# wwood/CoverM

Measured on AMD Instinct MI355X. Metric: aligned reads/s through coverm contig (mean trimmed_mean covered_fraction variance), higher is better.
Workload: dtype i32 depth / u64 sums / f32 estimators

## Files before the change

coverm_amd/csrc/pileup_kernels.hip.h:

```cpp
#pragma once
#include <hip/hip_runtime.h>
#include <stdint.h>

#define HSTC_FN __host__ __device__ __forceinline__
#include "hist_stats_core.h"
#include "scan_ops.hip.h"

namespace covk {

typedef unsigned long long u64;
typedef unsigned int u32;

constexpr u32 F_POS_UNSORTED = 1u;
constexpr u32 RW_SINGLE = 0u, RW_DOUBLE = 1u, RW_COMPLEX = 2u, RW_BUCKET = 3u;
constexpr u32 FAST_MAX_CAND = 8191u;
constexpr u32 TILE_F_GENERIC = 1u, TILE_F_SLOW = 2u;
constexpr u32 CX_MIN_OPS = 16;

struct DevContig {
    u64 n_primary, n_pass, n_nonsupp, sum_nm, sum_indel;
    double id_primary, id_nonsupp;
    u64 sum_d, sum_d2, cov_win, cov_full, proc_win;
    u64 hist_off;
    u32 first_rec, last_rec;
// ... 1029 lines not shown
    const u32 k0 = generic ? 0u : (rs + ID_CH - 1) / ID_CH, k1 = generic ? 0u : re / ID_CH;
    if (k0 >= k1) { serial(rs, re, true, true); }
    else {
        serial(rs, k0 * ID_CH, true, true);
        for (u32 kb = k0; kb < k1; kb += 64) {
            const u32 kk = kb + (u32)lane;
            IdChunk x;
            if (kk < k1) x = ch[kk]; else { x.tp = x.tn = 0; x.ep = x.en = ID_SERIAL; x.flags = 15u; }
            const u32 nb = min(64u, k1 - kb);
            auto run_stream = [&](double &S, const int e_l, const u64 t_l, const bool bad_l, const bool is_p) {
                u32 q = 0;
                while (q < nb) {
                    const u64 bits = (u64)__double_as_longlong(S);
                    const int e_cur = (int)((bits >> 52) & 0x7ff) - 1023;
                    const u64 m = (bits & 0xfffffffffffffull) | (1ull << 52);
                    const bool in_range = (u32)lane >= q && (u32)lane < nb;
                    const u64 P = wave_incl_scan_u64(in_range ? t_l : 0ull);
                    const bool fits = in_range && !bad_l && !(bits >> 63) && e_l == e_cur && t_l < (1ull << 53) &&
                                      P < (1ull << 53) && m + P < (1ull << 53);
                    const u64 failm = __ballot(in_range && !fits);
                    const u32 jstar = failm ? (u32)(__ffsll((long long)failm) - 1) : nb;
                    if (jstar > q) {
                        const u64 T = bcast_u64(P, (int)(jstar - 1));
                        S = __longlong_as_double((long long)((bits & 0xfff0000000000000ull) | ((m + T) & 0xfffffffffffffull)));
                    }
                    if (jstar < nb) serial((kb + jstar) * ID_CH, (kb + jstar + 1) * ID_CH, is_p, !is_p);
                    q = jstar + 1;
                }
            };
            if (identp != nullptr) run_stream(Sp, x.ep, x.tp, (x.flags & (1u | 4u)) != 0u, true);
            if (identn != nullptr) run_stream(Sn, x.en, x.tn, (x.flags & (2u | 8u)) != 0u, false);
        }
        serial(k1 * ID_CH, re, true, true);
    }
    if (lane == 0) { C->id_primary = Sp; C->id_nonsupp = Sn; }
}

__device__ __attribute__((noinline)) void hist_add_overflow(u32 *arena, u64 hoff, u32 hcap, DevGlobal *g, u32 d, u32 x) {
    if (d <= hcap) atomicAdd(&arena[hoff + d], x);
    else atomicOr(&g->internal_error, 1u);
}

struct PileupArgs {
    const u32 *tile_contig, *tile_start;
    const uint4 *desc;
    const uint2 *runs;
    const uint2 *cx_runs;
    Records r;
    DevContig *ctg;
    DevGlobal *g;
    u32 *hist_arena;
    u64 excl;
    int32_t *depth_out;
    const u64 *depth_off;
    u32 tile_base;
};


__device__ __forceinline__ void lds_fence() { asm volatile("s_waitcnt lgkmcnt(0)" ::: "memory"); }

constexpr int STREAM_TW = 1024, STREAM_HB = 512, STREAM_CAP = 512;

template <bool WANT_HIST, bool WRITE_DEPTH>
__global__ __launch_bounds__(256) void k_pileup_stream(PileupArgs a, u32 n_tiles, u32 chunk_tiles,
                                                       const u32 *__restrict__ tile_list, const u32 *__restrict__ n_list) {
    if (tile_list != nullptr) n_tiles = *n_list;
    constexpr int TW = STREAM_TW, HBW = STREAM_HB, CAP = STREAM_CAP, ROWS = TW / 64;
    extern __shared__ __attribute__((aligned(16))) char smem[];
    const int lane = threadIdx.x & 63, w = threadIdx.x >> 6;
    int *tile = reinterpret_cast<int *>(smem + (size_t)w * (TW * 4 + HBW * 4));
    u32 *lhist = reinterpret_cast<u32 *>(tile + TW);
    int4 *t4 = reinterpret_cast<int4 *>(tile);
    int2 *ent = reinterpret_cast<int2 *>(tile);
    const u32 wave_id = blockIdx.x * 4u + (u32)w, n_waves = gridDim.x * 4u;
    if (WANT_HIST) {
#pragma unroll
        for (int b = lane; b < HBW; b += 64) lhist[b] = 0u;
    }
    u64 sum_d = 0, sum_d2 = 0, proc_win = 0;
    u32 cov_w = 0, cov_f = 0, mn = 0xffffffffu, mx = 0;
    u32 cov_o = 0;
    u32 hbound = 0;
    int cur_c = -1;
    u64 hoff = 0; u32 hcap = 0;
    const u64 excl = a.excl;

    auto hist_add = [&](u32 d, u32 x) {
        if (__builtin_expect(d < (u32)HBW, 1)) atomicAdd(&lhist[d], x);
        else hist_add_overflow(a.hist_arena, hoff, hcap, a.g, d, x);
    };
    auto flush = [&]() {
        if (WANT_HIST) {
            if (cur_c >= 0) {
                lds_fence();
                for (u32 b = (u32)lane; b <= hbound; b += 64) {
                    const u32 x = lhist[b];
                    if (x) { atomicAdd(&a.hist_arena[hoff + b], x); lhist[b] = 0u; }
                }
                lds_fence();
                if (__any(cov_o != 0u)) {
                    const u32 co = wave_sum_u32(cov_o);
                    if (lane == 0) atomicAdd(&a.ctg[cur_c].cov_out, co);
                }
            }
            cov_o = 0; hbound = 0;
            return;
        }
        if (cur_c >= 0) {
            const u64 s1 = wave_sum_u64(sum_d), s2 = wave_sum_u64(sum_d2);
            const u32 c1 = wave_sum_u32(cov_w), c2 = wave_sum_u32(cov_f);
            const u32 m1 = wave_min_u32(mn), m2 = wave_max_u32(mx);
            DevContig *C = &a.ctg[cur_c];
            if (lane == 0) {
                if (s1) atomicAdd(&C->sum_d, s1);
                if (s2) atomicAdd(&C->sum_d2, s2);
                if (c1) atomicAdd(&C->cov_win, (u64)c1);
                if (c2) atomicAdd(&C->cov_full, (u64)c2);
                if (proc_win) {
                    atomicAdd(&C->proc_win, proc_win);
                    atomicMin(&C->min_d, m1);
                    atomicMax(&C->max_d, m2);
                }
            }
        }
        sum_d = sum_d2 = 0; proc_win = 0; cov_w = cov_f = 0; mn = 0xffffffffu; mx = 0;
    };

    auto load_runs = [&](const uint4 &d, uint2 &r0, uint2 &r1) {
        const u32 i0 = d.x + (u32)lane, i1 = i0 + 64u;
        r0 = i0 < d.y ? a.runs[i0] : make_uint2(0u, 0u);
        r1 = i1 < d.y ? a.runs[i1] : make_uint2(0u, 0u);
    };
    const u32 n_chunks = (n_tiles + chunk_tiles - 1) / chunk_tiles;
    u32 ch = wave_id < n_chunks ? wave_id : 0xffffffffu;
    while (ch != 0xffffffffu) {
        const u32 ch_next = ch + n_waves < n_chunks ? ch + n_waves : 0xffffffffu;
        const u32 t0 = a.tile_base + ch * chunk_tiles, t1 = a.tile_base + min((ch + 1) * chunk_tiles, n_tiles);
        for (u32 tq = t0; tq < t1; tq++) {
            const u32 t = tile_list != nullptr ? tile_list[tq] : tq;
            const uint4 ds = a.desc[2 * (size_t)t], dC1 = a.desc[2 * (size_t)t + 1];
            uint2 rw0, rw1;
            load_runs(ds, rw0, rw1);
            const u32 c = dC1.x, lo = dC1.y, L = ds.z;
            const u64 dbase = (WRITE_DEPTH && a.depth_off != nullptr) ? a.depth_off[c] : 0ull;
            const u32 cxo = dC1.z, cxn = dC1.w;
            if (ds.x >= ds.y && cxn == 0u) continue;
            const bool generic = ds.w & 1u;
            if ((int)c != cur_c) {
                flush();
                cur_c = (int)c;
                if (WANT_HIST) { hoff = a.ctg[c].hist_off; hcap = a.ctg[c].hist_cap; }
            }
            const u32 tlen_t = min((u32)TW, L - lo);
#pragma unroll
            for (int k = 0; k < TW / 256; k++) t4[k * 64 + lane] = make_int4(0, 0, 0, 0);
            lds_fence();
            const u32 hi = lo + TW;
            auto add_run = [&](u32 s, u32 e) {
                if (s < hi && e > lo) {
                    const u32 s0 = s > lo ? s - lo : 0u;
                    atomicAdd(&tile[s0], 1);
                    if (e < hi) atomicAdd(&tile[e - lo], -1);
                }
            };
            auto apply = [&](const uint2 rw, u32 i) {
                if (rw.y == 0u) return;
                if (generic && a.r.tid[i] != (int)c) return;
                const u32 type = rw.y >> 30;
                if (type <= RW_DOUBLE) {
                    const bool dbl = type == RW_DOUBLE;
                    const u32 l1 = dbl ? (rw.y & 1023u) : rw.y;
                    add_run(rw.x, rw.x + l1);
                    if (dbl) {
                        const u32 s2 = rw.x + l1 + ((rw.y >> 10) & 255u);
                        add_run(s2, s2 + ((rw.y >> 18) & 1023u));
                    }
                } else if (type == RW_COMPLEX) {
                    u32 cursor = (u32)a.r.pos[i];
                    const u32 c0 = a.r.cigar_off[i], c1 = a.r.cigar_off[i + 1];
                    for (u32 k = c0; k < c1; k++) {
                        const u32 wd = a.r.cigar[k];
                        const u32 op = wd & 15u, len = wd >> 4;
                        if (op == 0u || op == 7u || op == 8u) { add_run(cursor, cursor + len); cursor += len; }
                        else if (op == 2u || op == 3u) cursor += len;
                    }
                }
            };
            apply(rw0, ds.x + (u32)lane);
            apply(rw1, ds.x + 64u + (u32)lane);
            for (u32 i = ds.x + 128u + (u32)lane; i < ds.y; i += 64) apply(a.runs[i], i);
            for (u32 j = (u32)lane; j < cxn; j += 64) { const uint2 q = a.cx_runs[(u64)cxo + j]; add_run(q.x, q.y); }
            lds_fence();
            int x[ROWS];
            u32 E = 0;
#pragma unroll
            for (int j = 0; j < ROWS; j++) x[j] = tile[j * 64 + lane];
#pragma unroll
            for (int j = 0; j < ROWS; j++) E += (u32)__popcll(__ballot(x[j] != 0));
            const bool has_win = 2 * excl < (u64)L;
            const u32 ws = has_win ? (u32)excl : 0u, we = has_win ? (u32)(L - excl) : 0u;
            const u32 wst = max(ws, lo), wet = min(we, lo + tlen_t);
            const bool win_any = has_win && wst < wet;
            if (!WANT_HIST && win_any) proc_win += (u64)(wet - wst);
            if (WANT_HIST) hbound = max(hbound, min(ds.y - ds.x + cxn, (u32)HBW - 1u));

            if (!WRITE_DEPTH && E <= (u32)CAP) {
                u32 base = 0;
#pragma unroll
                for (int j = 0; j < ROWS; j++) {
                    const u64 m = __ballot(x[j] != 0);
                    if (x[j] != 0) {
                        const u32 rank = __builtin_amdgcn_mbcnt_hi((u32)(m >> 32), __builtin_amdgcn_mbcnt_lo((u32)m, 0u));
                        ent[base + rank] = make_int2(j * 64 + lane, x[j]);
                    }
                    base += (u32)__popcll(m);
                }
                lds_fence();
                const u32 wl0 = win_any ? wst - lo : 0u, wl1 = win_any ? wet - lo : 0u;
                if (lane == 0) {
                    const u32 en = min(E ? (u32)ent[0].x : tlen_t, tlen_t);
                    const u32 a1 = min(en, wl1);
                    if (a1 > wl0) { if (WANT_HIST) hist_add(0u, a1 - wl0); else mn = 0u; }
                }
                int carry = 0;
                u32 s1t = 0, s2t = 0;
                for (u32 e0 = 0; e0 < E; e0 += 64) {
                    const u32 e = e0 + (u32)lane;
                    const bool live = e < E;
                    const int2 en = live ? ent[e] : make_int2(0, 0);
                    const u32 nxt = (e + 1 < E) ? (u32)ent[e + 1].x : tlen_t;
                    const int inc = wave_incl_scan(en.y);
                    const int d = carry + inc;
                    carry += __builtin_amdgcn_readlane(inc, 63);
                    const u32 du = (u32)d;
                    const bool small = !__any(live && du >= 1024u);
                    if (live) {
                        const u32 s = min((u32)en.x, tlen_t), t_ = min(nxt, tlen_t);
                        const u32 a0 = max(s, wl0), a1 = min(t_, wl1);
                        if (WANT_HIST) {
                            const u32 len = a1 > a0 ? a1 - a0 : 0u;
                            if (d > 0) cov_o += (t_ - s) - len;
                            if (len) hist_add(du, len);
                        } else {
                            if (d > 0) cov_f += t_ - s;
                            if (a1 > a0) {
                                const u32 len = a1 - a0;
                                if (small) { s1t += __umul24(du, len); s2t += __umul24(__umul24(du, du), len); }
                                else { sum_d += (u64)du * len; sum_d2 += (u64)du * du * len; }
                                if (d > 0) cov_w += len;
                                mn = min(mn, du); mx = max(mx, du);
                            }
                        }
                    }
                }
                sum_d += s1t; sum_d2 += s2t;
            } else {
                int carry = 0;
#pragma unroll
                for (int j = 0; j < ROWS; j++) {
                    const int inc = wave_incl_scan(x[j]);
                    const int d = carry + inc;
                    carry += __builtin_amdgcn_readlane(inc, 63);
                    const u32 p = lo + (u32)(j * 64 + lane);
                    const u32 du = (u32)d;
                    if (p < L) {
                        if (WRITE_DEPTH) a.depth_out[dbase + p] = d;
                        const bool in_w = win_any && p >= wst && p < wet;
                        if (WANT_HIST) {
                            if (in_w) {
                                const u32 rel = p - wst;
                                if (x[j] != 0 && rel) { hist_add((u32)(d - x[j]), rel); hist_add(du, 0u - rel); }
                                if (p == wet - 1) hist_add(du, wet - wst);
                            } else cov_o += d > 0;
                        } else {
                            cov_f += d > 0;
                            if (in_w) {
                                sum_d += du;
                                sum_d2 += (u64)du * du;
                                cov_w += d > 0;
                                mn = min(mn, du); mx = max(mx, du);
                            }
                        }
                    }
                }
            }
        }
        flush();
        cur_c = -1;
        ch = ch_next;
    }
}

constexpr size_t pileup_stream_smem_bytes() { return (size_t)4 * ((size_t)STREAM_TW * 4 + STREAM_HB * 4); }

constexpr int FAST_TW = 1024, FAST_HB = 512;
constexpr int FAST_HB7 = 384;
constexpr size_t pileup_fast_smem_bytes(bool hist, int hb = FAST_HB, int tables = 2) { return (size_t)4 * ((size_t)FAST_TW * 2 * tables + (hist ? (size_t)hb * 4 : 0)); }

typedef short v2i16 __attribute__((ext_vector_type(2)));
typedef __attribute__((address_space(3))) u32 lds_u32_t;
__device__ __forceinline__ u32 lds_addr_of(const u32 *p) { return (u32)(uintptr_t)(lds_u32_t *)p; }
__device__ __forceinline__ void lds_atomic_add(u32 addr, u32 x) { (void)__hip_atomic_fetch_add((lds_u32_t *)(uintptr_t)addr, x, __ATOMIC_RELAXED, __HIP_MEMORY_SCOPE_WORKGROUP); }

template <bool WANT_HIST, int HB, int TABLES>
__device__ __forceinline__ void pileup_fast_body(const PileupArgs &a, u32 n_tiles, u32 chunk_tiles) {
    constexpr int TW = FAST_TW, HBW = HB;
    constexpr int DS = TABLES == 1 ? 2 : 0;
    constexpr size_t WB = (size_t)TW * 2 * TABLES + (WANT_HIST ? (size_t)HBW * 4 : 0);
    extern __shared__ __attribute__((aligned(16))) char smem[];
    const int lane = threadIdx.x & 63, w = threadIdx.x >> 6;
    u32 *S = reinterpret_cast<u32 *>(smem + (size_t)w * WB);
    u32 *E = TABLES == 2 ? S + TW / 2 : S;
    u32 *lhist = S + (TW / 2) * TABLES;
    uint4 *S4 = reinterpret_cast<uint4 *>(S), *E4 = reinterpret_cast<uint4 *>(E);
    const u32 wave_id = (u32)__builtin_amdgcn_readfirstlane((int)(blockIdx.x * 4u + (u32)w)), n_waves = gridDim.x * 4u;
    if (WANT_HIST) {
#pragma unroll
        for (int b = lane; b < HBW; b += 64) lhist[b] = 0u;
    }
    u64 sum_d = 0, sum_d2 = 0, proc_win = 0;
    u32 cov_w = 0, cov_f = 0, mn = 0xffffffffu, mx = 0;
    u32 cov_o = 0;
    int cur_c = -1;
    u64 hoff = 0; u32 hcap = 0;
    const u64 excl = a.excl;
    u32 hbound = 0;
    auto drain = [&]() {
        lds_fence();
        for (u32 b = (u32)lane; b <= hbound; b += 64) {
            const u32 x = lhist[b];
            if (x) { atomicAdd(&a.hist_arena[hoff + b], x); lhist[b] = 0u; }
        }
        lds_fence();
        hbound = 0;
    };

    auto hist_add = [&](u32 d, u32 x) {
        if (__builtin_expect(d < (u32)HBW, 1)) atomicAdd(&lhist[d], x);
        else hist_add_overflow(a.hist_arena, hoff, hcap, a.g, d, x);
    };
    auto flush = [&]() {
        if (WANT_HIST) {
            if (cur_c >= 0) {
                drain();
                if (__any(cov_o != 0u)) {
                    const u32 co = wave_sum_u32_dpp(cov_o);
                    if (lane == 0) atomicAdd(&a.ctg[cur_c].cov_out, co);
                }
            }
            cov_o = 0; hbound = 0;
            return;
        }
        if (cur_c >= 0) {
            const bool narrow = !__any((sum_d | sum_d2) >> 50);
            const u64 s1 = narrow ? wave_sum_u56(sum_d) : wave_sum_u64(sum_d), s2 = narrow ? wave_sum_u56(sum_d2) : wave_sum_u64(sum_d2);
            const u32 c1 = wave_sum_u32_dpp(cov_w), c2 = wave_sum_u32_dpp(cov_f);
            const u32 m1 = wave_min_u32_dpp(mn), m2 = wave_max_u32_dpp(mx);
            DevContig *C = &a.ctg[cur_c];
            if (lane == 0) {
                if (s1) atomicAdd(&C->sum_d, s1);
                if (s2) atomicAdd(&C->sum_d2, s2);
                if (c1) atomicAdd(&C->cov_win, (u64)c1);
                if (c2) atomicAdd(&C->cov_full, (u64)c2);
                if (proc_win) {
                    atomicAdd(&C->proc_win, proc_win);
                    atomicMin(&C->min_d, m1);
                    atomicMax(&C->max_d, m2);
                }
            }
        }
        sum_d = sum_d2 = 0; proc_win = 0; cov_w = cov_f = 0; mn = 0xffffffffu; mx = 0;
    };
    auto load_runs = [&](const uint4 &d, uint2 &r0, uint2 &r1) {
        const u32 i0 = d.x + (u32)lane, i1 = i0 + 64u;
        r0 = i0 < d.y ? a.runs[i0] : make_uint2(0u, 0u);
        r1 = i1 < d.y ? a.runs[i1] : make_uint2(0u, 0u);
    };
    const u32 n_chunks = (n_tiles + chunk_tiles - 1) / chunk_tiles;
    if (wave_id >= n_chunks) return;
    u32 ch = wave_id;
    u32 t = ch * chunk_tiles, t_end = min(t + chunk_tiles, n_tiles);
    uint4 ds = a.desc[2 * (size_t)(a.tile_base + t)], dC1 = a.desc[2 * (size_t)(a.tile_base + t) + 1];
    uint2 rw0, rw1;
    load_runs(ds, rw0, rw1);
    for (;;) {
        u32 tn = t + 1, tn_end = t_end, chn = ch;
        bool chunk_end = false;
        if (tn >= t_end) {
            chunk_end = true;
            chn = ch + n_waves;
            tn = chn < n_chunks ? chn * chunk_tiles : 0xffffffffu;
            tn_end = chn < n_chunks ? min(tn + chunk_tiles, n_tiles) : 0u;
        }
        const bool have_next = tn != 0xffffffffu;
        uint4 nds = make_uint4(0u, 0u, 0u, 0u), ndC1 = make_uint4(0u, 0u, 0u, 0u);
        if (have_next) { nds = a.desc[2 * (size_t)(a.tile_base + tn)]; ndC1 = a.desc[2 * (size_t)(a.tile_base + tn) + 1]; }

        const u32 c = dC1.x, lo = dC1.y, L = ds.z, cxo = dC1.z, cxn = dC1.w;
        const bool live = (ds.x < ds.y || cxn != 0u) && !(ds.w & TILE_F_SLOW);
        uint4 sv0, sv1, ev0, ev1;
        if (live) {
            if ((int)c != cur_c) {
                flush();
                cur_c = (int)c;
                if (WANT_HIST) { hoff = a.ctg[c].hist_off; hcap = a.ctg[c].hist_cap; }
            }
            const u32 zb = TABLES == 2 ? 0u : 0x80008000u;
            const uint4 z4 = make_uint4(zb, zb, zb, zb);
            S4[2 * lane] = z4; S4[2 * lane + 1] = z4;
            if (TABLES == 2) { E4[2 * lane] = z4; E4[2 * lane + 1] = z4; }
            asm volatile("" ::: "memory");
            const u32 hi = lo + TW;
            auto add_run = [&](u32 s, u32 e) {
                if (s < hi && e > lo) {
                    const u32 s0 = s > lo ? s - lo : 0u;
                    atomicAdd(&S[s0 >> 1], (1u << DS) << ((s0 & 1u) << 4));
                    if (e < hi) {
                        const u32 e0 = e - lo;
                        if (TABLES == 2) atomicAdd(&E[e0 >> 1], 1u << ((e0 & 1u) << 4)); else atomicSub(&E[e0 >> 1], (1u << DS) << ((e0 & 1u) << 4));
                    }
                }
            };
            auto apply = [&](const uint2 rw, u32 i) {
                if (rw.y == 0u) return;
                const u32 type = rw.y >> 30;
                if (type <= RW_DOUBLE) {
                    const bool dbl = type == RW_DOUBLE;
                    const u32 l1 = dbl ? (rw.y & 1023u) : rw.y;
                    add_run(rw.x, rw.x + l1);
                    if (dbl) {
                        const u32 s2 = rw.x + l1 + ((rw.y >> 10) & 255u);
                        add_run(s2, s2 + ((rw.y >> 18) & 1023u));
                    }
                } else if (type == RW_COMPLEX) {
                    u32 cursor = (u32)a.r.pos[i];
                    const u32 c0 = a.r.cigar_off[i], c1 = a.r.cigar_off[i + 1];
                    for (u32 k = c0; k < c1; k++) {
                        const u32 wd = a.r.cigar[k];
                        const u32 op = wd & 15u, len = wd >> 4;
                        if (op == 0u || op == 7u || op == 8u) { add_run(cursor, cursor + len); cursor += len; }
                        else if (op == 2u || op == 3u) cursor += len;
                    }
                }
            };
            apply(rw0, ds.x + (u32)lane);
            if (ds.y - ds.x > 64u) {
                apply(rw1, ds.x + 64u + (u32)lane);
                for (u32 i = ds.x + 128u + (u32)lane; i < ds.y; i += 64) apply(a.runs[i], i);
            }
            for (u32 j = (u32)lane; j < cxn; j += 64) { const uint2 q = a.cx_runs[(u64)cxo + j]; add_run(q.x, q.y); }
            asm volatile("" ::: "memory");
            sv0 = S4[2 * lane]; sv1 = S4[2 * lane + 1];
            if (TABLES == 2) { ev0 = E4[2 * lane]; ev1 = E4[2 * lane + 1]; }
        }
        uint2 nrw0 = make_uint2(0u, 0u), nrw1 = make_uint2(0u, 0u);
        if (have_next) load_runs(nds, nrw0, nrw1);

        if (live) {
            const u32 sw[8] = {sv0.x, sv0.y, sv0.z, sv0.w, sv1.x, sv1.y, sv1.z, sv1.w};
            u32 ew[8] = {0u, 0u, 0u, 0u, 0u, 0u, 0u, 0u};
            if (TABLES == 2) { ew[0] = ev0.x; ew[1] = ev0.y; ew[2] = ev0.z; ew[3] = ev0.w; ew[4] = ev1.x; ew[5] = ev1.y; ew[6] = ev1.z; ew[7] = ev1.w; }
            v2i16 dl[8];
#pragma unroll
            for (int k = 0; k < 8; k++) dl[k] = TABLES == 2 ? __builtin_bit_cast(v2i16, sw[k]) - __builtin_bit_cast(v2i16, ew[k]) : __builtin_bit_cast(v2i16, sw[k] ^ 0x80008000u);
            int net = 0;
            const v2i16 one2 = {1, 1};
#pragma unroll
            for (int k = 0; k < 8; k++) net = __builtin_amdgcn_sdot2(dl[k], one2, net, false);
            int d = wave_incl_scan(net) - net;

            const bool has_win = 2 * excl < (u64)L;
            const u32 tlen_t = min((u32)TW, L - lo);
            const u32 ws = has_win ? (u32)excl : 0u, we = has_win ? (u32)(L - excl) : 0u;
            const u32 wst = max(ws, lo), wet = min(we, lo + tlen_t);
            const bool win_any = has_win && wst < wet;
            if (!WANT_HIST && win_any) proc_win += (u64)(wet - wst);
            const bool interior = has_win && lo >= ws && lo + (u32)TW <= we;
            const u32 cand = ds.y - ds.x + cxn;
            const bool fast_tile = interior && cand < (u32)HBW;
            if (WANT_HIST) hbound = max(hbound, min(cand, (u32)HBW - 1u));
            if (WANT_HIST && fast_tile) {
                u32 seg0 = 0;
                u32 da = lds_addr_of(lhist) + ((u32)d << (2 - DS));
#pragma unroll
                for (int j = 0; j < 16; j++) {
                    const int dj = (j & 1) ? (int)dl[j >> 1].y : (int)dl[j >> 1].x;
                    if (j > 0 && dj != 0) { lds_atomic_add(da, (u32)j - seg0); seg0 = (u32)j; }
                    da += (u32)(dj << (2 - DS));
                }
                lds_atomic_add(da, 16u - seg0);
            } else if (WANT_HIST && cand < (u32)HBW) {
                const u32 p0 = lo + 16u * (u32)lane;
                const u32 wa = win_any ? min(max(wst, p0) - p0, 16u) : 0u, wb = win_any ? min(max(wet, p0) - p0, 16u) : 0u;
                const u32 le = min(max(L, p0) - p0, 16u);
                u32 seg0 = 0, covm = 0;
                const u32 da0 = lds_addr_of(lhist);
                u32 da = da0 + ((u32)d << (2 - DS));
#pragma unroll
                for (int j = 0; j < 16; j++) {
                    const int dj = (j & 1) ? (int)dl[j >> 1].y : (int)dl[j >> 1].x;
                    if (j > 0 && dj != 0) {
                        const u32 s_ = max(seg0, wa), e_ = min((u32)j, wb);
                        if (e_ > s_) lds_atomic_add(da, e_ - s_);
                        seg0 = (u32)j;
                    }
                    da += (u32)(dj << (2 - DS));
                    covm = covm + covm + (da != da0 ? 1u : 0u);
                }
                {
                    const u32 s_ = max(seg0, wa);
                    if (wb > s_) lds_atomic_add(da, wb - s_);
                }
                const u32 in_ctg = 0xffffu & ~(0xffffu >> le), in_win = (0xffffu >> wa) & ~(0xffffu >> wb);
                cov_o += (u32)__popc(covm & in_ctg & ~in_win);
            } else if (WANT_HIST) {
                const u32 p0 = lo + 16u * (u32)lane;
                u32 seg0 = 0;
                bool seg_open = false;
#pragma unroll 4
                for (int j = 0; j < 16; j++) {
                    const int dj = (j & 1) ? (int)dl[j >> 1].y : (int)dl[j >> 1].x;
                    const u32 p = p0 + (u32)j;
                    const bool in_w = win_any && p >= wst && p < wet;
                    if (seg_open && (dj != 0 || !in_w)) { hist_add((u32)d >> DS, (u32)j - seg0); seg_open = false; }
                    d += dj;
                    if (in_w) { if (!seg_open) { seg_open = true; seg0 = (u32)j; } }
                    else if (p < L) cov_o += d != 0 ? 1u : 0u;
                }
                if (seg_open) hist_add((u32)d >> DS, 16u - seg0);
            } else if (fast_tile) {
                u32 s1t = 0, s2t = 0, cv = 0;
#pragma unroll
                for (int j = 0; j < 16; j++) {
                    const int dj = (j & 1) ? (int)dl[j >> 1].y : (int)dl[j >> 1].x;
                    d += dj;
                    const u32 du = (u32)d >> DS;
                    s1t += du;
                    s2t = __umul24(du, du) + s2t;
                    cv += du != 0u ? 1u : 0u;
                    mn = min(mn, du); mx = max(mx, du);
                }
                sum_d += s1t; sum_d2 += s2t; cov_w += cv; cov_f += cv;
            } else {
                const u32 p0 = lo + 16u * (u32)lane;
#pragma unroll 4
                for (int j = 0; j < 16; j++) {
                    const int dj = (j & 1) ? (int)dl[j >> 1].y : (int)dl[j >> 1].x;
                    const u32 p = p0 + (u32)j;
                    const bool in_w = win_any && p >= wst && p < wet;
                    d += dj;
                    const u32 du = (u32)d >> DS;
                    if (p < L) cov_f += du != 0u ? 1u : 0u;
                    if (in_w) {
                        sum_d += du; sum_d2 += (u64)du * du;
                        cov_w += du != 0u ? 1u : 0u;
                        mn = min(mn, du); mx = max(mx, du);
                    }
                }
            }
        }
        if (chunk_end) { flush(); cur_c = -1; }
        if (!have_next) break;
        t = tn; t_end = tn_end; ch = chn; ds = nds; dC1 = ndC1; rw0 = nrw0; rw1 = nrw1;
    }
}

template <bool WANT_HIST>
__global__ __launch_bounds__(256) __attribute__((amdgpu_waves_per_eu(7, 7))) void k_pileup_fast(PileupArgs a, u32 n_tiles, u32 chunk_tiles) {
    pileup_fast_body<WANT_HIST, FAST_HB, 1>(a, n_tiles, chunk_tiles);
}
template <bool WANT_HIST>
__global__ __launch_bounds__(256) __attribute__((amdgpu_waves_per_eu(6, 6))) void k_pileup_fast2t(PileupArgs a, u32 n_tiles, u32 chunk_tiles) {
    pileup_fast_body<WANT_HIST, FAST_HB7, 2>(a, n_tiles, chunk_tiles);
}


struct DevEstimator { int kind; float min_frac; u64 excl; int exclude_mismatches; float trim_min, trim_max; u32 pad; };
static_assert(sizeof(DevEstimator) == 32, "DevEstimator mirrors cov_estimator");
constexpr u32 EST_MAX = 16;
struct EstParams { DevEstimator e[EST_MAX]; u32 n; u32 pad; };
enum { EST_MEAN = 0, EST_TRIMMED_MEAN = 1, EST_PILEUP_COUNTS = 2, EST_COVERED_FRACTION = 3, EST_COVERED_BASES = 4, EST_RPKM = 5, EST_TPM = 6,
       EST_VARIANCE = 7, EST_LENGTH = 8, EST_READ_COUNT = 9, EST_READS_PER_BASE = 10, EST_ANIR = 11 };

__device__ __forceinline__ float est_f32(u64 x) { return __ull2float_rn(x); }
__device__ __forceinline__ u64 est_f32_to_usize(float x) {
    if (!(x == x) || x <= 0.0f) return 0ull;
    if (x >= 18446744073709551616.0f) return ~0ull;
    return (u64)x;
}

template <typename BIN>
__device__ __forceinline__ u64 trimmed_total_wave(const BIN *__restrict__ bins, u32 nh, u64 bin0_extra, u64 min_index, u64 max_index) {
    const int lane = lane_id();
    u64 total = 0, carry = 0;
    int state = 0;
    for (u32 b = 0; b < nh && state < 2; b += 64) {
        const u32 i = b + (u32)lane;
        u64 n = i < nh ? (u64)bins[i] : 0ull;
        if (i == 0) n += bin0_extra;
        const u64 acc = carry + wave_incl_scan_u64(n);
        const bool valid = i < nh;
        int first = 0;
        if (state == 0) {
            const u64 sm = __ballot(valid && acc >= min_index);
            if (sm == 0) { carry = bcast_u64(acc, 63); continue; }
            const int ls = __ffsll((long long)sm) - 1;
            const u64 acc_s = bcast_u64(acc, ls);
            total = (acc_s > max_index ? max_index - min_index + 1 : acc_s - min_index + 1) * (u64)(b + (u32)ls);
            state = 1; first = ls + 1;
        }
        const u64 em = __ballot(valid && lane >= first && acc > max_index);
        const int le = em ? __ffsll((long long)em) - 1 : 64;
        u64 part = (valid && lane >= first && lane < le) ? n * (u64)i : 0ull;
        if (em && lane == le) {
            const u64 excess = acc - n;
            part = (max_index >= excess ? max_index - excess + 1 : 0ull) * (u64)i;
        }
        total += wave_sum_u64(part);
        if (em) state = 2;
        carry = bcast_u64(acc, 63);
    }
    return total;
}

struct EstEntry {
    u64 win_len, win_sum_d, win_sum_d2, win_covered, win_min_d, full_len, full_covered, n_reads, mismatches;
    u64 bin0_extra;
    u64 unobs_win, unobs_full;
    double identity;
    u32 nh;
};

constexpr u32 EST_SERIAL_BINS = 96;
template <bool LANES, typename BIN>
__device__ __forceinline__ bool estimate_entry(const EstEntry &E, const BIN *__restrict__ bins, bool in, bool live, const EstParams &P, float *__restrict__ o) {
#pragma clang fp contract(off)
    const int lane = lane_id();
    const u64 win_len = E.win_len, win_sum_d = E.win_sum_d, win_sum_d2 = E.win_sum_d2, win_covered = E.win_covered, win_min_d = E.win_min_d;
    const u64 full_len = E.full_len, full_covered = E.full_covered, n_reads = E.n_reads, mismatches = E.mismatches;
    const u32 nh = E.nh;
    const u64 bin0_extra = E.bin0_extra;
    bool nonzero = false;
    for (u32 k = 0; k < P.n; k++) {
        const DevEstimator e = P.e[k];
        float r = 0.0f;
        switch (e.kind) {
        case EST_MEAN: {
            const u64 T = win_len + E.unobs_win;
            if (T == 0 || (est_f32(win_covered) / est_f32(T)) < e.min_frac) break;
            const float num = e.exclude_mismatches ? est_f32(win_sum_d - mismatches) : est_f32(win_sum_d);
            r = num / est_f32(T);
            break;
        }
        case EST_TRIMMED_MEAN: {
            const u64 T = win_len + E.unobs_win;
            const bool walk = (!LANES || (in && live)) && T != 0 && !((est_f32(win_covered) / est_f32(T)) < e.min_frac) && win_covered != 0;
            const u64 min_index = est_f32_to_usize(__builtin_floorf(e.trim_min * est_f32(T)));
            const u64 max_index = est_f32_to_usize(__builtin_ceilf(e.trim_max * est_f32(T)));
            u64 total = 0;
            if (!LANES) {
                if (!walk) break;
                total = trimmed_total_wave(bins, nh, bin0_extra, min_index, max_index);
            } else {
                const bool serial = walk && nh <= EST_SERIAL_BINS;
                u64 acc = 0;
                int state = serial ? 0 : 2;
                for (u32 i = 0; __any(state < 2 && i < nh); i++) {
                    if (state < 2 && i < nh) {
                        u64 n = bins[i];
                        if (i == 0) n += bin0_extra;
                        acc += n;
                        if (state == 0) {
                            if (acc >= min_index) { total = (acc > max_index ? max_index - min_index + 1 : acc - min_index + 1) * (u64)i; state = 1; }
                        } else if (acc > max_index) {
                            const u64 excess = acc - n;
                            total += (max_index >= excess ? max_index - excess + 1 : 0ull) * (u64)i;
                            state = 2;
                        } else total += n * (u64)i;
                    }
                }
                for (u64 bm = __ballot(walk && !serial); bm != 0; bm &= bm - 1) {
                    const int l = __builtin_ctzll(bm);
                    const u64 bp = bcast_u64((u64)(uintptr_t)bins, l);
                    const u64 t = trimmed_total_wave(reinterpret_cast<const BIN *>((uintptr_t)bp), __builtin_amdgcn_readlane(nh, l), bcast_u64(bin0_extra, l),
                                                     bcast_u64(min_index, l), bcast_u64(max_index, l));
                    if (lane == l) total = t;
                }
                if (!walk) break;
            }
            r = est_f32(total) / est_f32(max_index - min_index);
            break;
        }
        case EST_COVERED_FRACTION: {
            const u64 T = full_len + E.unobs_full;
            if (T == 0 || (est_f32(full_covered) / est_f32(T)) < e.min_frac) break;
            r = est_f32(full_covered) / est_f32(T);
            break;
        }
        case EST_COVERED_BASES: {
            const u64 T = full_len + E.unobs_full;
            if (T == 0 || (est_f32(full_covered) / est_f32(T)) < e.min_frac) break;
            r = est_f32(full_covered);
            break;
        }
        case EST_RPKM: {
            const u64 T = full_len + E.unobs_full;
            if (T == 0 || (est_f32(full_covered) / est_f32(T)) < e.min_frac) break;
            r = est_f32(n_reads * 1000000000ull) / est_f32(T);
            break;
        }
        case EST_VARIANCE: {
            const u64 T = win_len + E.unobs_win;
            if (T == 0) break;
            if ((est_f32(win_covered) / est_f32(T)) < e.min_frac || T < 3 || win_len == 0) break;
            const u64 kk = E.unobs_win > 0 ? 0ull : win_min_d, N = T;
            const u64 ex = win_sum_d - kk * N;
            const u64 ex2 = win_sum_d2 - 2 * kk * win_sum_d + kk * kk * N;
            r = (est_f32(ex2) - est_f32(ex * ex) / est_f32(T)) / est_f32(T - 1);
            break;
        }
        case EST_LENGTH: r = est_f32(full_len + E.unobs_full); break;
        case EST_READ_COUNT: r = est_f32(n_reads); break;
        case EST_READS_PER_BASE: r = est_f32(n_reads) / est_f32(full_len + E.unobs_full); break;
        case EST_ANIR: r = n_reads == 0 ? 0.0f : (float)(E.identity / (double)n_reads); break;
        default: break;
        }
        if (!live) r = 0.0f;
        nonzero |= r > 0.0f;
        if (LANES) { if (in) o[k] = r; }
        else if (lane == 0) o[k] = r;
    }
    return nonzero;
}

__device__ __forceinline__ hstc::Stats hist_stats_wave(const u32 *__restrict__ bins, u64 n) {
    hstc::Stats s = hstc::of_bins(bins, n, (u32)lane_id(), 64u);
    const bool narrow = !__any((s.sum_d | s.sum_d2 | s.proc_win) >> 50);
    s.sum_d = narrow ? wave_sum_u56(s.sum_d) : wave_sum_u64(s.sum_d);
    s.sum_d2 = narrow ? wave_sum_u56(s.sum_d2) : wave_sum_u64(s.sum_d2);
    s.proc_win = narrow ? wave_sum_u56(s.proc_win) : wave_sum_u64(s.proc_win);
    s.cov_win = narrow ? wave_sum_u56(s.cov_win) : wave_sum_u64(s.cov_win);
    s.min_d = wave_min_u32_dpp(s.min_d); s.max_d = wave_max_u32_dpp(s.max_d);
    return s;
}
template <bool LANES>
__device__ __forceinline__ hstc::Stats hist_stats_derive(DevContig *C, const u32 *__restrict__ arena, bool act, bool has_win) {
    const int lane = lane_id();
    const u64 n = (act && has_win) ? (u64)C->hist_cap + 1 : 0ull;
    const u32 *bins = arena + (n ? C->hist_off : 0ull);
    hstc::Stats s = hstc::empty();
    if (!LANES) s = hist_stats_wave(bins, n);
    else {
        const bool serial = n <= (u64)EST_SERIAL_BINS;
        if (serial) s = hstc::of_bins(bins, n, 0u, 1u);
        for (u64 bm = __ballot(!serial); bm != 0; bm &= bm - 1) {
            const int l = __builtin_ctzll(bm);
            const u64 bp = bcast_u64((u64)(uintptr_t)bins, l);
            const hstc::Stats t = hist_stats_wave(reinterpret_cast<const u32 *>((uintptr_t)bp), bcast_u64(n, l));
            if (lane == l) s = t;
        }
    }
    if (act && (LANES || lane == 0)) {
        C->sum_d = s.sum_d; C->sum_d2 = s.sum_d2; C->cov_win = s.cov_win; C->proc_win = s.proc_win;
        C->cov_full = (u64)C->cov_out + s.cov_win;
        C->min_d = s.min_d; C->max_d = s.max_d;
    }
    return s;
}
template <bool LANES>
__global__ __launch_bounds__(256) void k_hist_stats(DevContig *ctg, u32 n_targets, const u32 *__restrict__ tlen, const uint8_t *__restrict__ mask, u64 excl,
                                                    const u32 *__restrict__ arena) {
    const u32 c_raw = LANES ? blockIdx.x * 256u + threadIdx.x : blockIdx.x * 4u + (threadIdx.x >> 6);
    if (!LANES && c_raw >= n_targets) return;
    const bool in = c_raw < n_targets;
    const u32 c = in ? c_raw : n_targets - 1u;
    DevContig *C = &ctg[c];
    const bool act = in && C->n_pass != 0 && (mask == nullptr || mask[c]);
    if (!LANES && !act) return;
    (void)hist_stats_derive<LANES>(C, arena, act, 2 * excl < (u64)tlen[c]);
}

template <bool LANES>
__device__ __forceinline__ void estimate_body(DevContig *ctg, u32 n_targets, const u32 *__restrict__ tlen, u64 excl,
                                              const u32 *__restrict__ arena, const EstParams &P, float *__restrict__ out, bool derive) {
    const int lane = lane_id();
    const u32 c_raw = LANES ? blockIdx.x * 256u + threadIdx.x : blockIdx.x * 4u + (threadIdx.x >> 6);
    if (!LANES && c_raw >= n_targets) return;
    const bool in = c_raw < n_targets;
    const u32 c = in ? c_raw : n_targets - 1u;
    DevContig *C = &ctg[c];
    float *o = out + (size_t)c * P.n;
    const bool touched = C->n_pass != 0;
    if (!LANES && !touched) { if ((u32)lane < P.n) o[lane] = 0.0f; return; }
    const u64 L = tlen[c];
    const bool has_win = 2 * excl < L;
    hstc::Stats S;
    u64 cov_full;
    if (derive) {
        S = hist_stats_derive<LANES>(C, arena, in && touched, has_win);
        cov_full = (u64)C->cov_out + S.cov_win;
    } else {
        S.sum_d = C->sum_d; S.sum_d2 = C->sum_d2; S.cov_win = C->cov_win; S.proc_win = C->proc_win; S.min_d = C->min_d; S.max_d = C->max_d;
        cov_full = C->cov_full;
    }
    EstEntry E;
    E.win_len = has_win ? L - 2 * excl : 0;
    E.win_sum_d = has_win ? S.sum_d : 0; E.win_sum_d2 = has_win ? S.sum_d2 : 0; E.win_covered = has_win ? S.cov_win : 0;
    E.win_min_d = has_win ? ((S.proc_win < E.win_len || S.min_d == 0xffffffffu) ? 0u : S.min_d) : 0xffffffffu;
    E.full_len = L; E.full_covered = cov_full; E.n_reads = C->n_primary; E.mismatches = C->sum_nm - C->sum_indel;
    E.nh = has_win ? S.max_d + 1u : 0u;
    E.bin0_extra = E.win_len - S.proc_win;
    E.unobs_win = 0; E.unobs_full = 0;
    E.identity = C->id_primary;
    (void)estimate_entry<LANES, u32>(E, arena + C->hist_off, in, touched, P, o);
}
__global__ __launch_bounds__(256) void k_estimate(DevContig *ctg, u32 n_targets, const u32 *__restrict__ tlen, u64 excl,
                                                  const u32 *__restrict__ arena, EstParams P, float *__restrict__ out, u32 derive) {
    estimate_body<false>(ctg, n_targets, tlen, excl, arena, P, out, derive != 0u);
}
__global__ __launch_bounds__(256) void k_estimate_lanes(DevContig *ctg, u32 n_targets, const u32 *__restrict__ tlen, u64 excl,
                                                        const u32 *__restrict__ arena, EstParams P, float *__restrict__ out, u32 derive) {
    estimate_body<true>(ctg, n_targets, tlen, excl, arena, P, out, derive != 0u);
}

struct DevInterval { u32 tid, pad; u64 start, end; };
struct DevIntervalStats { u64 win_sum_d, win_sum_d2, win_covered, full_covered; u32 win_min_d, win_max_d, hist_len, pad; u64 hist_off; };

__global__ __launch_bounds__(256) void k_interval_stats(const int32_t *__restrict__ depth, const u64 *__restrict__ depth_off,
                                                        const DevInterval *__restrict__ iv, u64 n, u64 excl,
                                                        DevIntervalStats *__restrict__ out) {
    const int lane = lane_id();
    const u64 wave = (u64)blockIdx.x * 4u + (threadIdx.x >> 6), n_waves = (u64)gridDim.x * 4u;
    for (u64 g = wave; g < n; g += n_waves) {
        const DevInterval I = iv[g];
        const int32_t *d = depth + depth_off[I.tid];
        const u64 len = I.end - I.start;
        const bool has_win = 2 * excl < len;
        const u64 ws = I.start + excl, we = has_win ? I.end - excl : ws;
        u64 s1 = 0, s2 = 0;
        u32 cw = 0, cf = 0, mn = 0xffffffffu, mx = 0;
        for (u64 p = I.start + (u64)lane; p < I.end; p += 64) {
            const u32 v = (u32)d[p];
            cf += v > 0u;
            if (has_win && p >= ws && p < we) { s1 += v; s2 += (u64)v * v; cw += v > 0u; mn = min(mn, v); mx = max(mx, v); }
        }
        s1 = wave_sum_u64(s1); s2 = wave_sum_u64(s2);
        cw = wave_sum_u32(cw); cf = wave_sum_u32(cf); mn = wave_min_u32(mn); mx = wave_max_u32(mx);
        if (lane == 0) {
            DevIntervalStats o;
            o.win_sum_d = s1; o.win_sum_d2 = s2; o.win_covered = cw; o.full_covered = cf;
            o.win_min_d = has_win ? mn : 0u; o.win_max_d = mx; o.hist_len = has_win ? mx + 1u : 0u; o.pad = 0; o.hist_off = 0;
            out[g] = o;
        }
    }
}

constexpr int IV_HB = 512;
__global__ __launch_bounds__(256) void k_interval_hist(const int32_t *__restrict__ depth, const u64 *__restrict__ depth_off,
                                                       const DevInterval *__restrict__ iv, u64 n, u64 excl,
                                                       const DevIntervalStats *__restrict__ st, unsigned long long *__restrict__ hist) {
    __shared__ u32 lh[4][IV_HB];
    const int lane = lane_id(), w = threadIdx.x >> 6;
    const u64 wave = (u64)blockIdx.x * 4u + (u64)w, n_waves = (u64)gridDim.x * 4u;
    for (int b = lane; b < IV_HB; b += 64) lh[w][b] = 0u;
    for (u64 g = wave; g < n; g += n_waves) {
        const DevInterval I = iv[g];
// ... 17 lines not shown
```

Baseline: 51.11 billion.

## Deepen tile prefetch pipeline with scalar descriptor loads and more run slots

Tile descriptors are now read as one uniform 32-byte scalar load, prefetched two tiles ahead, and contig histogram offsets are loaded a tile early through the scalar path. The number of prefetched run slots per lane rises to four for the single-table variant, and those loads are issued before the current tile's work rather than after it. The tail loop over extra runs gains software prefetch of the next element. The aim is to hide global-memory latency on descriptors and runs, at the cost of more registers held live in a kernel already pinned to a fixed waves-per-EU.

Result: no change. 50.70 billion (-0.8%).

```diff
diff --git a/coverm_amd/csrc/pileup_kernels.hip.h b/coverm_amd/csrc/pileup_kernels.hip.h
--- a/coverm_amd/csrc/pileup_kernels.hip.h
+++ b/coverm_amd/csrc/pileup_kernels.hip.h
@@ -1355,6 +1355,24 @@
 __device__ __forceinline__ u32 lds_addr_of(const u32 *p) { return (u32)(uintptr_t)(lds_u32_t *)p; }
 __device__ __forceinline__ void lds_atomic_add(u32 addr, u32 x) { (void)__hip_atomic_fetch_add((lds_u32_t *)(uintptr_t)addr, x, __ATOMIC_RELAXED, __HIP_MEMORY_SCOPE_WORKGROUP); }
 
+struct TileDesc { u32 x, y, L, w, c, lo, cxo, cxn; };
+typedef u32 u32x8_t __attribute__((ext_vector_type(8)));
+__device__ __forceinline__ TileDesc tile_desc_uniform(const uint4 *desc, u32 t) {
+    typedef __attribute__((address_space(4))) const u32x8_t cu32x8;
+    const u32x8_t v = *(cu32x8 *)(uintptr_t)(desc + 2 * (size_t)t);
+    TileDesc d;
+    d.x = v[0]; d.y = v[1]; d.L = v[2]; d.w = v[3]; d.c = v[4]; d.lo = v[5]; d.cxo = v[6]; d.cxn = v[7];
+    return d;
+}
+__device__ __forceinline__ void contig_hist_uniform(const DevContig *ctg, u32 c, u64 &hoff, u32 &hcap) {
+    typedef __attribute__((address_space(4))) const u64 cu64;
+    typedef __attribute__((address_space(4))) const u32 cu32;
+    const uintptr_t p = (uintptr_t)(ctg + c);
+    hoff = *(cu64 *)(p + offsetof(DevContig, hist_off));
+    hcap = *(cu32 *)(p + offsetof(DevContig, hist_cap));
+}
+constexpr int fast_slots(int tables) { return tables == 1 ? 4 : 2; }
+
 template <bool WANT_HIST, int HB, int TABLES>
 __device__ __forceinline__ void pileup_fast_body(const PileupArgs &a, u32 n_tiles, u32 chunk_tiles) {
     constexpr int TW = FAST_TW, HBW = HB;
@@ -1424,39 +1442,52 @@
         }
         sum_d = sum_d2 = 0; proc_win = 0; cov_w = cov_f = 0; mn = 0xffffffffu; mx = 0;
     };
-    auto load_runs = [&](const uint4 &d, uint2 &r0, uint2 &r1) {
-        const u32 i0 = d.x + (u32)lane, i1 = i0 + 64u;
-        r0 = i0 < d.y ? a.runs[i0] : make_uint2(0u, 0u);
-        r1 = i1 < d.y ? a.runs[i1] : make_uint2(0u, 0u);
+    constexpr int NS = fast_slots(TABLES);
+    constexpr bool EARLY = TABLES == 1;
+    auto load_runs = [&](const TileDesc &d, bool ok, uint2 (&r)[NS]) {
+#pragma unroll
+        for (int k = 0; k < NS; k++) {
+            const u32 i = d.x + (u32)(64 * k + lane);
+            r[k] = a.runs[(ok && i < d.y) ? i : 0u];
+        }
     };
     const u32 n_chunks = (n_tiles + chunk_tiles - 1) / chunk_tiles;
     if (wave_id >= n_chunks) return;
-    u32 ch = wave_id;
-    u32 t = ch * chunk_tiles, t_end = min(t + chunk_tiles, n_tiles);
-    uint4 ds = a.desc[2 * (size_t)(a.tile_base + t)], dC1 = a.desc[2 * (size_t)(a.tile_base + t) + 1];
-    uint2 rw0, rw1;
-    load_runs(ds, rw0, rw1);
+    auto succ = [&](u32 &t_, u32 &te_, u32 &ch_) -> bool {
+        if (t_ + 1 < te_) { t_++; return true; }
+        if (n_chunks - ch_ <= n_waves) return false;
+        ch_ += n_waves;
+        t_ = ch_ * chunk_tiles; te_ = min(t_ + chunk_tiles, n_tiles);
+        return true;
+    };
+    const uint4 *desc_w = a.desc + 2 * (size_t)a.tile_base;
+    u32 pt = wave_id * chunk_tiles, pte = min(pt + chunk_tiles, n_tiles), pch = wave_id;
+    TileDesc ds = tile_desc_uniform(desc_w, pt), nds = ds, nnds = ds;
+    bool chunk_end = pt + 1 >= pte, n_chunk_end = false, nn_chunk_end = false;
+    bool have_next = succ(pt, pte, pch);
+    if (have_next) { nds = tile_desc_uniform(desc_w, pt); n_chunk_end = pt + 1 >= pte; }
+    u64 hoff_t = 0, n_hoff = 0; u32 hcap_t = 0, n_hcap = 0;
+    if (WANT_HIST) contig_hist_uniform(a.ctg, ds.c, hoff_t, hcap_t);
+    uint2 rw[NS], nrw[NS];
+    load_runs(ds, true, rw);
+    asm volatile("" :: "s"(nds.c), "s"(hcap_t), "s"((u32)hoff_t));
     for (;;) {
-        u32 tn = t + 1, tn_end = t_end, chn = ch;
-        bool chunk_end = false;
-        if (tn >= t_end) {
-            chunk_end = true;
-            chn = ch + n_waves;
-            tn = chn < n_chunks ? chn * chunk_tiles : 0xffffffffu;
-            tn_end = chn < n_chunks ? min(tn + chunk_tiles, n_tiles) : 0u;
-        }
-        const bool have_next = tn != 0xffffffffu;
-        uint4 nds = make_uint4(0u, 0u, 0u, 0u), ndC1 = make_uint4(0u, 0u, 0u, 0u);
-        if (have_next) { nds = a.desc[2 * (size_t)(a.tile_base + tn)]; ndC1 = a.desc[2 * (size_t)(a.tile_base + tn) + 1]; }
-
-        const u32 c = dC1.x, lo = dC1.y, L = ds.z, cxo = dC1.z, cxn = dC1.w;
+        bool have_nn = false;
+        if (have_next) {
+            have_nn = succ(pt, pte, pch);
+            if (have_nn) { nnds = tile_desc_uniform(desc_w, pt); nn_chunk_end = pt + 1 >= pte; }
+            if (WANT_HIST) contig_hist_uniform(a.ctg, nds.c, n_hoff, n_hcap);
+        }
+        if (EARLY) load_runs(nds, have_next, nrw);
+
+        const u32 c = ds.c, lo = ds.lo, L = ds.L, cxo = ds.cxo, cxn = ds.cxn;
         const bool live = (ds.x < ds.y || cxn != 0u) && !(ds.w & TILE_F_SLOW);
         uint4 sv0, sv1, ev0, ev1;
         if (live) {
             if ((int)c != cur_c) {
                 flush();
                 cur_c = (int)c;
-                if (WANT_HIST) { hoff = a.ctg[c].hist_off; hcap = a.ctg[c].hist_cap; }
+                if (WANT_HIST) { hoff = hoff_t; hcap = hcap_t; }
             }
             const u32 zb = TABLES == 2 ? 0u : 0x80008000u;
             const uint4 z4 = make_uint4(zb, zb, zb, zb);
@@ -1475,7 +1506,7 @@
                 }
             };
             auto apply = [&](const uint2 rw, u32 i) {
-                if (rw.y == 0u) return;
+                if (rw.y == 0u || i >= ds.y) return;
                 const u32 type = rw.y >> 30;
                 if (type <= RW_DOUBLE) {
                     const bool dbl = type == RW_DOUBLE;
@@ -1496,18 +1527,33 @@
                     }
                 }
             };
-            apply(rw0, ds.x + (u32)lane);
-            if (ds.y - ds.x > 64u) {
-                apply(rw1, ds.x + 64u + (u32)lane);
-                for (u32 i = ds.x + 128u + (u32)lane; i < ds.y; i += 64) apply(a.runs[i], i);
+            const u32 n_cand = ds.y - ds.x;
+            apply(rw[0], ds.x + (u32)lane);
+            if (n_cand > 64u) {
+                apply(rw[1], ds.x + 64u + (u32)lane);
+                if (NS > 2 && n_cand > 128u) {
+                    apply(rw[NS > 2 ? 2 : 0], ds.x + 128u + (u32)lane);
+                    if (n_cand > 192u) apply(rw[NS > 2 ? 3 : 0], ds.x + 192u + (u32)lane);
+                }
+                if (n_cand > 64u * (u32)NS) {
+                    u32 i = ds.x + 64u * (u32)NS + (u32)lane;
+                    uint2 q = i < ds.y ? a.runs[i] : make_uint2(0u, 0u);
+                    for (u32 left = n_cand - 64u * (u32)NS; ; left -= 64u) {
+                        const u32 in_ = i + 64u;
+                        uint2 qn = make_uint2(0u, 0u);
+                        if (left > 64u && in_ < ds.y) qn = a.runs[in_];
+                        apply(q, i);
+                        if (left <= 64u) break;
+                        q = qn; i = in_;
+                    }
+                }
             }
             for (u32 j = (u32)lane; j < cxn; j += 64) { const uint2 q = a.cx_runs[(u64)cxo + j]; add_run(q.x, q.y); }
             asm volatile("" ::: "memory");
             sv0 = S4[2 * lane]; sv1 = S4[2 * lane + 1];
             if (TABLES == 2) { ev0 = E4[2 * lane]; ev1 = E4[2 * lane + 1]; }
         }
-        uint2 nrw0 = make_uint2(0u, 0u), nrw1 = make_uint2(0u, 0u);
-        if (have_next) load_runs(nds, nrw0, nrw1);
+        if (!EARLY) load_runs(nds, have_next, nrw);
 
         if (live) {
             const u32 sw[8] = {sv0.x, sv0.y, sv0.z, sv0.w, sv1.x, sv1.y, sv1.z, sv1.w};
@@ -1614,7 +1660,10 @@
         }
         if (chunk_end) { flush(); cur_c = -1; }
         if (!have_next) break;
-        t = tn; t_end = tn_end; ch = chn; ds = nds; dC1 = ndC1; rw0 = nrw0; rw1 = nrw1;
+        ds = nds; nds = nnds; chunk_end = n_chunk_end; n_chunk_end = nn_chunk_end; have_next = have_nn;
+        hoff_t = n_hoff; hcap_t = n_hcap;
+#pragma unroll
+        for (int k = 0; k < NS; k++) rw[k] = nrw[k];
     }
 }
 
```
